# lkeegan/blockCG

Measured on AMD Instinct MI355X. Metric: SBCGrQ lattice-site iterations/sec (iterations/sec x global volume), fp64, higher is better.
Workload: dtype f64; 1 GPU; SBCGrQ V=64x64x64x64 (64x64x64x64 per GPU), m=16, 4 shifts, mass=0.001, fixed-work (eps=0); m=16, transport=none, half_volume_solves=False, memory_ladder_rung=whole tmp

## Files before the change

blockcg_amd/csrc/mfma_common.hpp:

```cpp
#pragma once
#include <hip/hip_runtime.h>

#include <cstdlib>

#include "kernels.hpp"
#include "kernels_mfma.hpp"

#include <type_traits>

namespace bcg {

namespace {

typedef double d4 __attribute__((ext_vector_type(4)));
typedef double dv2 __attribute__((ext_vector_type(2)));

__device__ __forceinline__ d4 mfma(double a, double b, d4 c) {
  return __builtin_amdgcn_mfma_f64_16x16x4f64(a, b, c, 0, 0, 0);
}
__device__ __forceinline__ d4 mfma_nega(double a, double b, d4 c) {
  return __builtin_amdgcn_mfma_f64_16x16x4f64(a, b, c, 0, 0, 1);
}

__device__ __forceinline__ double2 ld_nt(const double2* p) {
  const dv2 v = __builtin_nontemporal_load(reinterpret_cast<const dv2*>(p));
  return make_double2(v.x, v.y);
}
__device__ __forceinline__ void st_sc1(double2* p, double2 v) {
  dv2 w;
  w.x = v.x;
  w.y = v.y;
  asm volatile("global_store_dwordx4 %0, %1, off sc1" : : "v"(p), "v"(w));
}

template <int M>
struct MatLds {
  static constexpr int LD = 2 * M + 1;
  static constexpr int DOUBLES = M * LD;
};

template <int M>
__device__ __forceinline__ void stage_matrix(double* Ml, const double2* __restrict__ Cg, int tid, int nthreads) {
  for (int e = tid; e < M * M; e += nthreads) {
    const int i = e % M, jo = e / M;
    const double2 v = Cg[e];
    Ml[i * MatLds<M>::LD + 2 * jo] = v.x;
    Ml[i * MatLds<M>::LD + 2 * jo + 1] = v.y;
  }
}

template <int M>
struct Tile {
  double2 v[M / 4];
};

template <int M>
__device__ __forceinline__ void tile_load(Tile<M>& t, const double2* __restrict__ f, int64_t row, int kq, bool ok) {
  const double2* p = f + row * M + kq;
#pragma unroll
  for (int s = 0; s < M / 4; ++s) t.v[s] = ok ? p[4 * s] : make_double2(0.0, 0.0);
}
template <int M>
__device__ __forceinline__ void tile_store(const Tile<M>& t, double2* __restrict__ f, int64_t row, int kq, bool ok) {
  double2* p = f + row * M + kq;
  if (ok) {
#pragma unroll
    for (int s = 0; s < M / 4; ++s) p[4 * s] = t.v[s];
  }
}
#ifdef BCG_ROWS_ALWAYS_FULL
#define BCG_ROW_OK(row, rows) true
#else
#define BCG_ROW_OK(row, rows) ((row) < (rows))
#endif


template <int M>
struct Acc {
  d4 a[M / 8];
};
template <int M>
__device__ __forceinline__ void acc_from_tile(Acc<M>& A, const Tile<M>& t) {
#pragma unroll
  for (int s = 0; s < M / 4; ++s) {
    A.a[s >> 2][s & 3] = t.v[s].x;
    A.a[(M / 4 + s) >> 2][(M / 4 + s) & 3] = t.v[s].y;
  }
}
template <int M>
__device__ __forceinline__ void acc_zero(Acc<M>& A) {
#pragma unroll
  for (int q = 0; q < M / 8; ++q) A.a[q] = d4{0.0, 0.0, 0.0, 0.0};
}
template <int M>
__device__ __forceinline__ void tile_from_acc(Tile<M>& t, const Acc<M>& A) {
#pragma unroll
  for (int s = 0; s < M / 4; ++s) {
    t.v[s].x = A.a[s >> 2][s & 3];
    t.v[s].y = A.a[(M / 4 + s) >> 2][(M / 4 + s) & 3];
  }
}

template <int M>
__device__ __forceinline__ void rmul_acc(Acc<M>& A, const Tile<M>& in, const double* Ml, int lane) {
  static_assert(M == 8 || M == 16 || M == 32, "MFMA right-multiply is instantiated for m = 8, 16, 32");
  constexpr int LD = MatLds<M>::LD;
  const int kq = lane >> 4;
  const int ar = lane & 15;
#pragma unroll
  for (int T = 0; T < (M + 7) / 8; ++T) {
    const int q_o = 4 * T + (ar >> 2);
    const int ri_o = q_o / (M / 4);
    const int s_o = q_o % (M / 4);
    const int j_o = 4 * s_o + (ar & 3);
    const double* base = Ml + kq * LD + 2 * j_o;
#pragma unroll
    for (int s_i = 0; s_i < M / 4; ++s_i) {
      const double a_same = base[s_i * 4 * LD + 0];
      const double a_cross = base[s_i * 4 * LD + 1];
      if (M >= 16) {
        if ((4 * T) / (M / 4) == 0) {
          A.a[T] = mfma(a_same, in.v[s_i].x, A.a[T]);
          A.a[T] = mfma_nega(a_cross, in.v[s_i].y, A.a[T]);
        } else {
          A.a[T] = mfma(a_cross, in.v[s_i].x, A.a[T]);
          A.a[T] = mfma(a_same, in.v[s_i].y, A.a[T]);
        }
      } else {
        const double c_re = ri_o ? a_cross : a_same;
        const double c_im = ri_o ? a_same : -a_cross;
        A.a[T] = mfma(c_re, in.v[s_i].x, A.a[T]);
        A.a[T] = mfma(c_im, in.v[s_i].y, A.a[T]);
      }
    }
  }
}

template <int M>
__device__ __forceinline__ void rmul_acc2(Acc<M>& A1, const double* Ml1, Acc<M>& A2, const double* Ml2, const Tile<M>& in,
                                          int lane) {
  constexpr int LD = MatLds<M>::LD;
  const int kq = lane >> 4;
  const int ar = lane & 15;
#pragma unroll
  for (int T = 0; T < (M + 7) / 8; ++T) {
    const int q_o = 4 * T + (ar >> 2);
    const int ri_o = q_o / (M / 4);
    const int s_o = q_o % (M / 4);
    const int j_o = 4 * s_o + (ar & 3);
    const int off = kq * LD + 2 * j_o;
#pragma unroll
    for (int s_i = 0; s_i < M / 4; ++s_i) {
      const double a1s = Ml1[off + s_i * 4 * LD], a1c = Ml1[off + s_i * 4 * LD + 1];
      const double a2s = Ml2[off + s_i * 4 * LD], a2c = Ml2[off + s_i * 4 * LD + 1];
      if (M >= 16) {
        if ((4 * T) / (M / 4) == 0) {
          A1.a[T] = mfma(a1s, in.v[s_i].x, A1.a[T]);
          A2.a[T] = mfma(a2s, in.v[s_i].x, A2.a[T]);
          A1.a[T] = mfma_nega(a1c, in.v[s_i].y, A1.a[T]);
          A2.a[T] = mfma_nega(a2c, in.v[s_i].y, A2.a[T]);
        } else {
          A1.a[T] = mfma(a1c, in.v[s_i].x, A1.a[T]);
          A2.a[T] = mfma(a2c, in.v[s_i].x, A2.a[T]);
          A1.a[T] = mfma(a1s, in.v[s_i].y, A1.a[T]);
          A2.a[T] = mfma(a2s, in.v[s_i].y, A2.a[T]);
        }
      } else {
        const double c1r = ri_o ? a1c : a1s, c1i = ri_o ? a1s : -a1c;
        const double c2r = ri_o ? a2c : a2s, c2i = ri_o ? a2s : -a2c;
        A1.a[T] = mfma(c1r, in.v[s_i].x, A1.a[T]);
        A2.a[T] = mfma(c2r, in.v[s_i].x, A2.a[T]);
        A1.a[T] = mfma(c1i, in.v[s_i].y, A1.a[T]);
        A2.a[T] = mfma(c2i, in.v[s_i].y, A2.a[T]);
      }
    }
  }
}

template <int M>
struct GramAcc {
  d4 re[(M / 16) * (M / 16)];
  d4 im[(M / 16) * (M / 16)];
};
template <int M>
__device__ __forceinline__ void gram_zero(GramAcc<M>& G) {
#pragma unroll
  for (int q = 0; q < (M / 16) * (M / 16); ++q) {
    G.re[q] = d4{0.0, 0.0, 0.0, 0.0};
    G.im[q] = d4{0.0, 0.0, 0.0, 0.0};
  }
}
template <int M>
__device__ __forceinline__ void gram_step(GramAcc<M>& G, const double2* a, const double2* b) {
  constexpr int JB = M / 16;
#pragma unroll
  for (int ja = 0; ja < JB; ++ja)
#pragma unroll
    for (int jb = 0; jb < JB; ++jb) {
      const int q = ja * JB + jb;
      G.re[q] = mfma(a[ja].x, b[jb].x, G.re[q]);
      G.re[q] = mfma(a[ja].y, b[jb].y, G.re[q]);
      G.im[q] = mfma(a[ja].x, b[jb].y, G.im[q]);
      G.im[q] = mfma_nega(a[ja].y, b[jb].x, G.im[q]);
    }
}

__device__ __forceinline__ void st_partial(double2* p, double2 v, bool wt) {
  if (wt) st_sc1(p, v);
  else *p = v;
}
template <int M, int NW>
__device__ __forceinline__ void gram_block_store(const GramAcc<M>& G, double* red, double2* __restrict__ partials, int tid,
                                                 bool wt = false) {
  constexpr int JB = M / 16;
  const int wave = tid >> 6, lane = tid & 63;
#pragma unroll
  for (int q = 0; q < JB * JB; ++q) {
    __syncthreads();
#pragma unroll
    for (int r = 0; r < 4; ++r) {
      red[(wave * 8 + r) * 64 + lane] = G.re[q][r];
      red[(wave * 8 + 4 + r) * 64 + lane] = G.im[q][r];
    }
    __syncthreads();
    for (int e = tid; e < 4 * 64; e += NW * 64) {
      const int l = e & 63, r = (e >> 6) & 3;
      double sr = 0.0, si = 0.0;
#pragma unroll
      for (int w = 0; w < NW; ++w) {
        sr += red[(w * 8 + r) * 64 + l];
        si += red[(w * 8 + 4 + r) * 64 + l];
      }
      const int i = 16 * (q / JB) + (l >> 4) + 4 * r, j = 16 * (q % JB) + (l & 15);
      st_partial(partials + static_cast<int64_t>(blockIdx.x) * (M * M) + j * M + i, make_double2(sr, si), wt);
    }
  }
}

template <int NW>
__device__ __forceinline__ void gram_block_store_fold8(const GramAcc<16>& G, double* red, double2* __restrict__ partials, int tid,
                                                       bool wt = false) {
  constexpr int FR = 8;
  const int wave = tid >> 6, lane = tid & 63;
  __syncthreads();
#pragma unroll
  for (int r = 0; r < 4; ++r) {
    red[((wave * FR) + r) * 64 + lane] = G.re[0][r];
    red[((wave * FR) + 4 + r) * 64 + lane] = G.im[0][r];
  }
  __syncthreads();
  for (int e = tid; e < 4 * 64; e += NW * 64) {
    const int l = e & 63, r = e >> 6;
    if (r >= 2 || (l & 15) >= 8) continue;
    double sr = 0.0, si = 0.0;
#pragma unroll
    for (int w = 0; w < NW; ++w) {
      sr += red[((w * FR) + r) * 64 + l] + red[((w * FR) + r + 2) * 64 + l + 8];
      si += red[((w * FR) + 4 + r) * 64 + l] + red[((w * FR) + 4 + r + 2) * 64 + l + 8];
    }
    const int i = (l >> 4) + 4 * r, j = l & 7;
    st_partial(partials + static_cast<int64_t>(blockIdx.x) * 64 + j * 8 + i, make_double2(sr, si), wt);
  }
}


__device__ __forceinline__ double2 sum_sc1(const double2* p, int64_t stride, int n) {
  double sr = 0.0, si = 0.0;
  int k = 0;
  for (; k + 8 <= n; k += 8) {
    dv2 r0, r1, r2, r3, r4, r5, r6, r7;
    const double2* q = p + static_cast<int64_t>(k) * stride;
    asm volatile("global_load_dwordx4 %0, %1, off sc1" : "=v"(r0) : "v"(q));
    asm volatile("global_load_dwordx4 %0, %1, off sc1" : "=v"(r1) : "v"(q + stride));
    asm volatile("global_load_dwordx4 %0, %1, off sc1" : "=v"(r2) : "v"(q + 2 * stride));
    asm volatile("global_load_dwordx4 %0, %1, off sc1" : "=v"(r3) : "v"(q + 3 * stride));
    asm volatile("global_load_dwordx4 %0, %1, off sc1" : "=v"(r4) : "v"(q + 4 * stride));
    asm volatile("global_load_dwordx4 %0, %1, off sc1" : "=v"(r5) : "v"(q + 5 * stride));
    asm volatile("global_load_dwordx4 %0, %1, off sc1" : "=v"(r6) : "v"(q + 6 * stride));
    asm volatile("global_load_dwordx4 %0, %1, off sc1" : "=v"(r7) : "v"(q + 7 * stride));
    asm volatile("s_waitcnt vmcnt(0)" : "+v"(r0), "+v"(r1), "+v"(r2), "+v"(r3), "+v"(r4), "+v"(r5), "+v"(r6), "+v"(r7) : : "memory");
    sr += r0.x; si += r0.y; sr += r1.x; si += r1.y; sr += r2.x; si += r2.y; sr += r3.x; si += r3.y;
    sr += r4.x; si += r4.y; sr += r5.x; si += r5.y; sr += r6.x; si += r6.y; sr += r7.x; si += r7.y;
  }
  for (; k < n; ++k) {
    dv2 r;
    asm volatile("global_load_dwordx4 %0, %1, off sc1\n\ts_waitcnt vmcnt(0)" : "=v"(r) : "v"(p + static_cast<int64_t>(k) * stride) : "memory");
    sr += r.x;
    si += r.y;
  }
  return make_double2(sr, si);
}
template <int NV>
__device__ __forceinline__ void gram_fold(const GramFold& gf, double2* __restrict__ partials, int tid, int nthreads) {
  if (gf.out == nullptr) return;
  __shared__ int s_role;
  const int nb = gridDim.x, g = blockIdx.x & 7;
  const int in_group = (nb - g + 7) >> 3;
  asm volatile("s_waitcnt vmcnt(0)" ::: "memory");
  __syncthreads();
  if (tid == 0) {
    const unsigned t = __hip_atomic_fetch_add(gf.tickets + g, 1u, __ATOMIC_RELAXED, __HIP_MEMORY_SCOPE_AGENT);
    s_role = t == static_cast<unsigned>(in_group - 1) ? 1 : 0;
  }
  __syncthreads();
  if (!s_role) return;
  double2* const level2 = partials + static_cast<int64_t>(nb) * NV;
  for (int v = tid; v < NV; v += nthreads)
    st_sc1(level2 + g * NV + v, sum_sc1(partials + static_cast<int64_t>(g) * NV + v, static_cast<int64_t>(8) * NV, in_group));
  const int groups = nb < 8 ? nb : 8;
  asm volatile("s_waitcnt vmcnt(0)" ::: "memory");
  __syncthreads();
  if (tid == 0) {
    const unsigned t = __hip_atomic_fetch_add(gf.tickets + 8, 1u, __ATOMIC_RELAXED, __HIP_MEMORY_SCOPE_AGENT);
    s_role = t == static_cast<unsigned>(groups - 1) ? 2 : 0;
  }
  __syncthreads();
  if (s_role != 2) return;
  for (int v = tid; v < NV; v += nthreads) gf.out[v] = sum_sc1(level2 + v, NV, groups);
  if (tid < 9) gf.tickets[tid] = 0u;
}

inline int grid_tiles(int64_t ntiles, int per_block, int cap) {
  int64_t g = (ntiles + per_block - 1) / per_block;
  if (g > cap) g = cap;
  if (g < 1) g = 1;
  return static_cast<int>(g);
}

template <typename K>
void allow_lds(K kernel, size_t bytes) {
  if (bytes > 48 * 1024) (void)hipFuncSetAttribute(reinterpret_cast<const void*>(kernel), hipFuncAttributeMaxDynamicSharedMemorySize, static_cast<int>(bytes));
}

}
}
```

Baseline: 359.2 million site-iter/s.

## Use Gauss 3-multiply complex product in MFMA right-multiply for m=16

Replaces the 4-real-MFMA complex matrix right-multiply with Gauss's 3-multiplication trick for m=16, in both the single and paired accumulate paths. A shared product K = c*(x+y) is accumulated separately and folded into the real and imaginary accumulators at the end. This cuts MFMA count per complex block by a quarter, in exchange for extra VALU adds, an extra accumulator register set, and slightly different fp64 rounding. It can be disabled with BCG_COMPLEX_4M.

```diff
diff --git a/blockcg_amd/csrc/mfma_common.hpp b/blockcg_amd/csrc/mfma_common.hpp
--- a/blockcg_amd/csrc/mfma_common.hpp
+++ b/blockcg_amd/csrc/mfma_common.hpp
@@ -101,12 +101,47 @@
   }
 }
 
+#ifdef BCG_COMPLEX_4M
+template <int M>
+constexpr bool kGauss3M = false;
+#else
+template <int M>
+constexpr bool kGauss3M = M == 16;
+#endif
+
+__device__ __forceinline__ void rmul_gauss_fold(d4& AR, d4& AI, const d4& K) {
+#pragma unroll
+  for (int i = 0; i < 4; ++i) {
+    AR[i] += K[i];
+    AI[i] += K[i];
+  }
+}
+
 template <int M>
 __device__ __forceinline__ void rmul_acc(Acc<M>& A, const Tile<M>& in, const double* Ml, int lane) {
   static_assert(M == 8 || M == 16 || M == 32, "MFMA right-multiply is instantiated for m = 8, 16, 32");
   constexpr int LD = MatLds<M>::LD;
   const int kq = lane >> 4;
   const int ar = lane & 15;
+  if constexpr (kGauss3M<M>) {
+    constexpr int H = M / 16;
+#pragma unroll
+    for (int h = 0; h < H; ++h) {
+      const int j_o = 4 * (4 * h + (ar >> 2)) + (ar & 3);
+      const double* base = Ml + kq * LD + 2 * j_o;
+      d4 K = d4{0.0, 0.0, 0.0, 0.0};
+#pragma unroll
+      for (int s_i = 0; s_i < M / 4; ++s_i) {
+        const double c = base[s_i * 4 * LD + 0];
+        const double d = base[s_i * 4 * LD + 1];
+        K = mfma(c, in.v[s_i].x + in.v[s_i].y, K);
+        A.a[h] = mfma_nega(c + d, in.v[s_i].y, A.a[h]);
+        A.a[H + h] = mfma(d - c, in.v[s_i].x, A.a[H + h]);
+      }
+      rmul_gauss_fold(A.a[h], A.a[H + h], K);
+    }
+    return;
+  }
 #pragma unroll
   for (int T = 0; T < (M + 7) / 8; ++T) {
     const int q_o = 4 * T + (ar >> 2);
@@ -142,6 +177,29 @@
   constexpr int LD = MatLds<M>::LD;
   const int kq = lane >> 4;
   const int ar = lane & 15;
+  if constexpr (kGauss3M<M>) {
+    constexpr int H = M / 16;
+#pragma unroll
+    for (int h = 0; h < H; ++h) {
+      const int off = kq * LD + 2 * (4 * (4 * h + (ar >> 2)) + (ar & 3));
+      d4 K1 = d4{0.0, 0.0, 0.0, 0.0}, K2 = d4{0.0, 0.0, 0.0, 0.0};
+#pragma unroll
+      for (int s_i = 0; s_i < M / 4; ++s_i) {
+        const double c1 = Ml1[off + s_i * 4 * LD], d1 = Ml1[off + s_i * 4 * LD + 1];
+        const double c2 = Ml2[off + s_i * 4 * LD], d2 = Ml2[off + s_i * 4 * LD + 1];
+        const double xs = in.v[s_i].x + in.v[s_i].y;
+        K1 = mfma(c1, xs, K1);
+        K2 = mfma(c2, xs, K2);
+        A1.a[h] = mfma_nega(c1 + d1, in.v[s_i].y, A1.a[h]);
+        A2.a[h] = mfma_nega(c2 + d2, in.v[s_i].y, A2.a[h]);
+        A1.a[H + h] = mfma(d1 - c1, in.v[s_i].x, A1.a[H + h]);
+        A2.a[H + h] = mfma(d2 - c2, in.v[s_i].x, A2.a[H + h]);
+      }
+      rmul_gauss_fold(A1.a[h], A1.a[H + h], K1);
+      rmul_gauss_fold(A2.a[h], A2.a[H + h], K2);
+    }
+    return;
+  }
 #pragma unroll
   for (int T = 0; T < (M + 7) / 8; ++T) {
     const int q_o = 4 * T + (ar >> 2);
```

After: 371.3 million site-iter/s (median of 6 runs). 1.03x the previous value.
